# CILAB-MA/gpudrive_lab

Hardware: AMD Instinct MI355X
Metric: agent-steps/sec at 1024 worlds x 64 agents; achieved HBM GB/s on obs kernel (higher is better)
Workload: dtype f32

## Files before the change

### gpudrive_lab_amd/csrc/engine.cpp

```cpp
#include <hip/hip_runtime.h>

#include <algorithm>
#include <cmath>
#include <cstdlib>
#include <cstdio>
#include <cstring>
#include <map>
#include <memory>
#include <stdexcept>
#include <atomic>
#include <exception>
#include <string>
#include <thread>
#include <vector>

#include "engine.hpp"
#include "gd_math.hpp"
#include "scene.hpp"
#ifdef GD_CLOCKS
namespace gd { void set_clocks_read(unsigned long long *out); void step_clocks_read(unsigned long long *out); }
#endif
#ifndef GD_GRID_MIN_CELL
#define GD_GRID_MIN_CELL 16.f
#endif
// ... 100 lines not shown
    size_t lin_cap = 0;
    int32_t *d_row_of_slot = nullptr, *d_slot_of_row = nullptr, *d_row_count = nullptr;
    int32_t *d_lin_list = nullptr, *d_lin_list_dyn = nullptr;
    std::vector<std::vector<int32_t>> w_resp;
    bool full_pass_next = false;
    int64_t lin_static_agents = 0;
    int64_t host_skipped = 0;
    bool rk_possible = false;
    bool rk_alloc = false;

    bool ensure_rank_buffers() {
        if (rk_alloc) return true;
        const size_t WA = static_cast<size_t>(W) * A;
        const size_t first = internal.size();
        try {
            if (std::getenv("GPUDRIVE_RANK_ALLOC_FAIL") != nullptr) {
                d.rk_E = alloc_internal<uint16_t>(WA * GD_RANK_CAP + 64);
                d.rk_spc = alloc_internal<uint16_t>(WA * GD_RANK_SPL);
                throw HipError("GPUDRIVE_RANK_ALLOC_FAIL: simulated allocation failure of the rank replay's buffers");
            }
            d.rk_E = alloc_internal<uint16_t>(WA * GD_RANK_CAP + 64);
            d.rk_spc = alloc_internal<uint16_t>(WA * GD_RANK_SPL);
            d.rk_kt = alloc_internal<float>(WA * GD_RANK_KT);
            d.rk_heap = alloc_internal<uint32_t>(WA * GD_RANK_HEAP_DW);
            d.rk_cpe = alloc_internal<uint16_t>(WA * GD_RANK_NCP);
            d.rk_n = alloc_internal<int32_t>(WA);
            d.rk_fallback = alloc_internal<int32_t>(WA / 32);
            d.rk_streak = alloc_internal<int32_t>(WA / 32);
            d.cp_road = alloc_internal<uint16_t>(2 * WA * GD_RANK_NCP);
            d.cp_T = alloc_internal<float>(2 * WA * GD_RANK_NCP);
            d.cp_hdr = alloc_internal<float4>(2 * WA);
            d.rk_words = alloc_internal<uint32_t>(WA * GD_RANK_NCH);
            d.rk_tl = alloc_internal<float>(WA);
            d.rk_hist = alloc_internal<int32_t>(544);
            d.rk_ticket = alloc_internal<int32_t>(WA);
            d.rk_order = alloc_internal<int32_t>(WA);
            d.rk_list = alloc_internal<int32_t>(8 * WA);
            d.rk_nlong = static_cast<int>(std::max<size_t>(WA / 4, 64));
            d.rk_longlist = alloc_internal<int32_t>(d.rk_nlong);
            d.rk_longslot = alloc_internal<int32_t>(WA);
            d.rk_E_long = alloc_internal<uint16_t>(static_cast<size_t>(d.rk_nlong) * GD_RANK_CAP_LONG + 64);
            d.rk_kt_long = alloc_internal<float>(static_cast<size_t>(d.rk_nlong) * GD_RANK_KT_LONG);
        } catch (const HipError &) {
            (void)hipGetLastError();
            for (size_t k = first; k < internal.size(); k++) (void)hipFree(internal[k]);
            internal.resize(first);
            rk_possible = false;
            d.rk_on = 0;
            d.rk_nlong = 0;
            d.rk_E = nullptr; d.rk_spc = nullptr; d.rk_kt = nullptr; d.rk_heap = nullptr; d.rk_cpe = nullptr; d.rk_n = nullptr;
            d.rk_fallback = nullptr; d.rk_streak = nullptr; d.cp_road = nullptr; d.cp_T = nullptr; d.cp_hdr = nullptr;
            d.rk_words = nullptr; d.rk_tl = nullptr; d.rk_hist = nullptr; d.rk_ticket = nullptr; d.rk_order = nullptr;
            d.rk_list = nullptr; d.rk_longlist = nullptr; d.rk_longslot = nullptr; d.rk_E_long = nullptr; d.rk_kt_long = nullptr;
            return false;
        }
        rk_alloc = true;
        return true;
    }
    bool timing = false;
    std::vector<EventPair> ev_pool[gd::KERNEL_TIMED];
    size_t ev_head[gd::KERNEL_TIMED] = {};
    size_t ev_used[gd::KERNEL_TIMED] = {};
    double ev_ms[gd::KERNEL_TIMED] = {};
    int64_t ev_launches[gd::KERNEL_TIMED] = {};

    ~gd_sim() {
        (void)hipDeviceSynchronize();
// ... 49 lines not shown
    void launch(int which, bool move, hipStream_t stream_override = nullptr) {
        hipStream_t stream = stream_override ? stream_override : this->stream;
        const bool timed = timing && which < gd::KERNEL_TIMED && !d.gate_any;
        EventPair ep{};
        if (timed) {
            if (ev_used[which] == ev_pool[which].size()) collect_timing(which, ev_pool[which].size() / 2);
            ep = ev_pool[which][(ev_head[which] + ev_used[which]) % ev_pool[which].size()];
            ev_used[which]++;
            HIP_CHECK(hipEventRecord(ep.start, stream));
        }
        if (which == gd::KERNEL_BEV) gd::launch_bev(d, stream);
        else if (which == gd::KERNEL_LIDAR) gd::launch_lidar(d, stream);
        else gd::launch_kernel(d, stream, which, move);
        if (timed) HIP_CHECK(hipEventRecord(ep.stop, stream));
        HIP_CHECK(hipGetLastError());
    }

    hipGraphExec_t step_graph = nullptr;
    int64_t stat_graph_steps = 0, stat_plain_steps = 0, stat_captures = 0;
    bool graph_ok = std::getenv("GPUDRIVE_NO_GRAPH") == nullptr;

    void drop_graph() {
        if (step_graph) {
            (void)hipGraphExecDestroy(step_graph);
            step_graph = nullptr;
        }
    }

    void choose_set_schedule() {
        d.set_apw = 2;
        d.set_fused_rows = 1;
        if (const char *e = std::getenv("GPUDRIVE_SET_FUSED_ROWS")) d.set_fused_rows = std::atoi(e) != 0 ? 1 : 0;
        if (const char *e = std::getenv("GPUDRIVE_SET_AGENTS_PER_WAVE")) d.set_apw = std::min(32, std::max(1, std::atoi(e)));
    }

    void step() {
        if (full_pass_next) {
            full_pass_next = false;
            d.lin_dyn_off = 1;
            d.bev_all_dirty = 1;
            try {
                run_rest(true);
            } catch (...) {
                d.lin_dyn_off = 0;
                d.bev_all_dirty = 0;
                throw;
            }
            d.lin_dyn_off = 0;
            d.bev_all_dirty = 0;
            stat_plain_steps++;
            return;
        }
        if (params.roadObservationAlgorithm != GD_ROADS_K_NEAREST && d.lin_on && d.pose_skip && !params.disableClassicalObs)
            host_skipped += lin_static_agents;
        if (!graph_ok || timing || stream == nullptr) {
            run_rest(true);
            stat_plain_steps++;
            return;
        }
        if (!step_graph) {
            hipGraph_t g = nullptr;
            if (hipStreamBeginCapture(stream, hipStreamCaptureModeThreadLocal) != hipSuccess) {
                (void)hipGetLastError();
                graph_ok = false;
                run_rest(true);
                return;
// ... 509 lines not shown
        std::vector<int32_t> co(ncell);
        std::vector<uint16_t> ci(nitem);
        std::vector<float> cxy(nitem * 2);
        std::vector<uint16_t> cpos(nitem);
        for (int w = 0; w < W; w++) {
            std::copy(w_rcell_off[w].begin(), w_rcell_off[w].end(), co.begin() + w_rgrid[w].cell_base);
            std::copy(w_rcell_items[w].begin(), w_rcell_items[w].end(), ci.begin() + w_rgrid[w].item_base);
            for (size_t k = 0; k < w_rcell_items[w].size(); k++) {
                const size_t r = w_rcell_items[w][k], o = (static_cast<size_t>(w_rgrid[w].item_base) + k) * 2;
                cxy[o] = w_xy[w][2 * r];
                cxy[o + 1] = w_xy[w][2 * r + 1];
                cpos[static_cast<size_t>(w_rgrid[w].item_base) + r] = static_cast<uint16_t>(k);
            }
        }
        if (ncell) HIP_CHECK(hipMemcpy(d_rcell_off, co.data(), ncell * sizeof(int32_t), hipMemcpyHostToDevice));
        if (nitem) HIP_CHECK(hipMemcpy(d_rcell_items, ci.data(), nitem * sizeof(uint16_t), hipMemcpyHostToDevice));
        if (nitem) HIP_CHECK(hipMemcpy(d_rcell_xy, cxy.data(), nitem * 2 * sizeof(float), hipMemcpyHostToDevice));
        if (nitem) HIP_CHECK(hipMemcpy(d_rcell_pos, cpos.data(), nitem * sizeof(uint16_t), hipMemcpyHostToDevice));
        d.rcell_xy = static_cast<const float2 *>(d_rcell_xy);
        d.rcell_pos = static_cast<const uint16_t *>(d_rcell_pos);
        HIP_CHECK(hipMemcpy(const_cast<gd::GridHdr *>(d.rgrid), w_rgrid.data(), sizeof(gd::GridHdr) * W, hipMemcpyHostToDevice));
        d.rcell_off = static_cast<const int32_t *>(d_rcell_off);
        d.rcell_items = static_cast<const uint16_t *>(d_rcell_items);
        std::vector<float> prev(static_cast<size_t>(W) * A * 4, 0.f);
        for (size_t i = 0; i < static_cast<size_t>(W) * A; i++) prev[i * 4 + 2] = INFINITY;
        HIP_CHECK(hipMemcpy(d.knn_prev, prev.data(), prev.size() * sizeof(float), hipMemcpyHostToDevice));
    }

    void reset_rank_state() {
        HIP_CHECK(hipMemset(d.cp_hdr, 0, sizeof(float4) * 2 * static_cast<size_t>(W) * A));
        HIP_CHECK(hipMemset(d.rk_fallback, 0, sizeof(int32_t) * (static_cast<size_t>(W) * A / 32)));
        HIP_CHECK(hipMemset(d.rk_streak, 0, sizeof(int32_t) * (static_cast<size_t>(W) * A / 32)));
        HIP_CHECK(hipMemset(d.rk_hist, 0, sizeof(int32_t) * GD_RANK_AUDIT));
    }

    void do_reset(const std::vector<int32_t> &flags) {
        upload_flags(d.reset_flags, flags);
        reset_flagged(false);
    }

    void reset_flagged(bool gated) {
        d.gate_any = gated ? 1 : 0;
        if (!gated) full_pass_next = false;
        try {
            launch(gd::KERNEL_RESET, false);
            run_rest(false);
        } catch (...) {
            d.gate_any = 0;
            throw;
        }
        d.gate_any = 0;
    }
};

namespace {

template <typename F>
int guarded(F &&f) {
    try {
        f();
        return GD_OK;
    } catch (const HipError &e) {
        return fail(GD_ERR_DEVICE, e.what());
    } catch (const std::invalid_argument &e) {
        const std::string m = e.what();
        return fail(m.find("cannot open") != std::string::npos ? GD_ERR_IO : GD_ERR_INVALID, m);
// ... 62 lines not shown
        s->w_boxes.resize(W);
        s->w_grid.resize(W);
        s->w_cell_off.resize(W);
        s->w_cell_items.resize(W);
        s->w_rgrid.resize(W);
        s->w_rcell_off.resize(W);
        s->w_rcell_items.resize(W);
        for (int id = 0; id < GD_T_COUNT; id++) {
            if (id == GD_T_BEV && !cfg->alloc_bev && !cfg->external[id]) continue;
            const int64_t bytes = spec_bytes(tensor_spec(id, W, A));
            if (cfg->external[id]) {
                s->exported[id] = cfg->external[id];
            } else {
                HIP_CHECK(hipMalloc(&s->exported[id], bytes));
                s->owned[id] = true;
            }
            HIP_CHECK(hipMemset(s->exported[id], 0, bytes));
        }
        gd::DevSim &d = s->d;
        d.W = W;
        d.A = A;
        d.p = *params;
        d.knn_order = cfg->knn_order;
        d.split_partner = (s->stream != nullptr && std::getenv("GPUDRIVE_SPLIT_PARTNER") != nullptr) ? 1 : 0;
        HIP_CHECK(hipStreamCreateWithFlags(&s->side, hipStreamNonBlocking));
        HIP_CHECK(hipEventCreateWithFlags(&s->ev_fork, hipEventDisableTiming));
        HIP_CHECK(hipEventCreateWithFlags(&s->ev_join, hipEventDisableTiming));
        d.step_dbg = 0;
#ifdef GD_DIAG
        if (const char *e = std::getenv("GPUDRIVE_STEP_DBG")) d.step_dbg = std::atoi(e);
#endif
        {
            (void)hipDeviceGetAttribute(&s->cu_count, hipDeviceAttributeMultiprocessorCount, cfg->device_id);
            d.set_fused_rows = 0;
            d.set_apw = 16;
        }
        d.lidar_half_angle = cfg->lidar_half_angle;
        {
            const float r = params->observationRadius;
            float k = r * r;
            while (k > 0.f && sqrtf(k) > r) k = std::nextafterf(k, 0.f);
            while (sqrtf(std::nextafterf(k, INFINITY)) <= r) k = std::nextafterf(k, INFINITY);
            d.radius_key_max = r >= 0.f ? k : -1.f;
        }
        d.action = static_cast<float *>(s->exported[GD_T_ACTION]);
        d.reward = static_cast<float *>(s->exported[GD_T_REWARD]);
        d.done = static_cast<int32_t *>(s->exported[GD_T_DONE]);
        d.info = static_cast<int32_t *>(s->exported[GD_T_INFO]);
        d.self_obs = static_cast<float *>(s->exported[GD_T_SELF_OBS]);
        d.abs_obs = static_cast<float *>(s->exported[GD_T_ABS_OBS]);
        d.partner = static_cast<float *>(s->exported[GD_T_PARTNER_OBS]);
        d.agent_map = static_cast<float *>(s->exported[GD_T_AGENT_MAP_OBS]);
        d.map_obs = static_cast<float *>(s->exported[GD_T_MAP_OBS]);
        d.lidar = static_cast<float *>(s->exported[GD_T_LIDAR]);
        d.bev = static_cast<float *>(s->exported[GD_T_BEV]);
        d.steps = static_cast<uint32_t *>(s->exported[GD_T_STEPS_REMAINING]);
        d.shape = static_cast<int32_t *>(s->exported[GD_T_SHAPE]);
        d.controlled = static_cast<int32_t *>(s->exported[GD_T_CONTROLLED_STATE]);
        d.resp_export = static_cast<int32_t *>(s->exported[GD_T_RESPONSE_TYPE]);
        d.traj = static_cast<float *>(s->exported[GD_T_EXPERT_TRAJECTORY]);
        d.means = static_cast<float *>(s->exported[GD_T_WORLD_MEANS]);
        d.metadata = static_cast<int32_t *>(s->exported[GD_T_METADATA]);
        d.deleted = static_cast<int32_t *>(s->exported[GD_T_DELETED_AGENTS]);
        d.map_name = static_cast<int32_t *>(s->exported[GD_T_MAP_NAME]);
        d.scenario_id = static_cast<int32_t *>(s->exported[GD_T_SCENARIO_ID]);
        const size_t WA = static_cast<size_t>(W) * A;
// ... 419 lines not shown
    });
}

int gd_stat(gd_sim *s, int32_t which, int64_t *out) {
#ifdef GD_CLOCKS
    if (s && out && which >= 22 && which <= 29) {
        static unsigned long long clk[8];
        if (which == 22) gd::set_clocks_read(clk);
        *out = (int64_t)clk[which - 22];
        return GD_OK;
    }
#endif
#ifdef GD_CLOCKS
    if (s && out && which >= 32 && which <= 43) {
        static unsigned long long clk[12];
        if (which == 32) gd::step_clocks_read(clk);
        *out = (int64_t)clk[which - 32];
        return GD_OK;
    }
#endif
#ifdef GD_CLOCKS
    if (s && out && which >= 1000 && which < 1256) {
        *out = 0;
        if (s->rk_alloc) {
            int32_t v = 0;
            (void)hipStreamSynchronize(s->stream);
            if (hipMemcpy(&v, s->d.rk_hist + 256 + (which - 1000), sizeof(v), hipMemcpyDeviceToHost) != hipSuccess)
                return fail(GD_ERR_DEVICE, "gd_stat: reading the replay clocks failed");
            *out = v;
        }
        return GD_OK;
    }
#endif
#if defined(GD_DIAG) || defined(GD_CLOCKS)
    constexpr int32_t kLastStat = 20;
#else
    constexpr int32_t kLastStat = 7;
#endif
    if (s && out && which == 30) {
        std::vector<unsigned long long> v(GD_SKIP_SLOTS, 0);
        (void)hipStreamSynchronize(s->stream);
        if (hipMemcpy(v.data(), s->d.stat_skipped, sizeof(unsigned long long) * v.size(), hipMemcpyDeviceToHost) != hipSuccess ||
            hipMemset(s->d.stat_skipped, 0, sizeof(unsigned long long) * v.size()) != hipSuccess)
            return fail(GD_ERR_DEVICE, "gd_stat: reading the skip counters failed");
        unsigned long long sum = 0;
        for (unsigned long long x : v) sum += x;
        *out = static_cast<int64_t>(sum) + s->host_skipped;
        s->host_skipped = 0;
        return GD_OK;
    }
    if (s && out && which == 31) {
        int32_t c = 0;
        (void)hipStreamSynchronize(s->stream);
        if (hipMemcpy(&c, s->d.bev_count, sizeof(c), hipMemcpyDeviceToHost) != hipSuccess)
            return fail(GD_ERR_DEVICE, "gd_stat: reading the raster count failed");
        *out = c;
        return GD_OK;
    }
    if (s && out && which == 44) {
        std::vector<int32_t> f(static_cast<size_t>(s->W) * s->A), n(static_cast<size_t>(s->W) * 2);
        (void)hipStreamSynchronize(s->stream);
        if (hipMemcpy(f.data(), s->d.lidar_dirty, sizeof(int32_t) * f.size(), hipMemcpyDeviceToHost) != hipSuccess ||
            hipMemcpy(n.data(), s->d.shape, sizeof(int32_t) * n.size(), hipMemcpyDeviceToHost) != hipSuccess)
            return fail(GD_ERR_DEVICE, "gd_stat: reading the LiDAR flags failed");
        int64_t c = 0;
        for (int w = 0; w < s->W; w++)
            for (int a = 0; a < n[static_cast<size_t>(w) * 2] && a < s->A; a++) c += f[static_cast<size_t>(w) * s->A + a] != 0;
        *out = c;
        return GD_OK;
    }
    if (s && out && which == 45) {
        unsigned long long v = 0;
        (void)hipStreamSynchronize(s->stream);
        if (hipMemcpy(&v, s->d.bad_actions, sizeof(v), hipMemcpyDeviceToHost) != hipSuccess)
            return fail(GD_ERR_DEVICE, "gd_stat: reading the action counter failed");
        *out = static_cast<int64_t>(v);
        return GD_OK;
    }
    if (s && out && which == 46) {
        unsigned long long v = 0;
        (void)hipStreamSynchronize(s->stream);
        if (hipMemcpy(&v, s->d.warm_count, sizeof(v), hipMemcpyDeviceToHost) != hipSuccess)
            return fail(GD_ERR_DEVICE, "gd_stat: reading the warm-up counter failed");
        *out = static_cast<int64_t>(v);
        return GD_OK;
    }
    if (s && out && which == 21) {
        *out = 0;
        if (s->rk_alloc) {
            int32_t v = 0;
            (void)hipStreamSynchronize(s->stream);
            if (hipMemcpy(&v, s->d.rk_hist + GD_RANK_AUDIT, sizeof(v), hipMemcpyDeviceToHost) != hipSuccess)
                return fail(GD_ERR_DEVICE, "gd_stat: reading the audit counter failed");
            *out = v;
        }
        return GD_OK;
    }
    if (!s || !out || which < 0 || which > kLastStat) return fail(GD_ERR_INVALID, "gd_stat: bad argument");
#if defined(GD_DIAG) || defined(GD_CLOCKS)
    if (which >= 8) {
        *out = 0;
        if (s->rk_alloc) {
            int32_t v = 0;
            (void)hipStreamSynchronize(s->stream);
            (void)hipMemcpy(&v, s->d.rk_hist + 514 + (which - 8), sizeof(v), hipMemcpyDeviceToHost);
            (void)hipMemset(s->d.rk_hist + 514 + (which - 8), 0, sizeof(v));
            *out = v;
        }
        return GD_OK;
    }
#endif
    if (which == 7) {
        *out = s->d.rk_on;
        return GD_OK;
    }
    *out = which == 0 ? s->stat_graph_steps : which == 1 ? s->stat_plain_steps : which == 2 ? s->stat_captures
         : which == 3 ? s->d.set_fused_rows : which == 4 ? s->d.set_apw : which == 5 ? s->d.live_count : GD_MAP_OBS_AW;
// ... 152 lines not shown
```

### gpudrive_lab_amd/csrc/engine.hpp

```cpp
#pragma once
#include <hip/hip_runtime.h>

#include <cstdint>

#include "../../include/gpudrive_amd.h"

#ifndef GD_MAP_OBS_AW
#define GD_MAP_OBS_AW 32
#endif

#define GD_RANK_CAP 1280
#define GD_RANK_NCP 40
#define GD_RANK_HEAP_DW 104
#define GD_RANK_CAP_LONG 2560
#define GD_RANK_KT_LONG 164
#define GD_RH_LONG 537
#define GD_RANK_NCH 320
#define GD_RANK_SPL 256
#define GD_RANK_KT 84
#define GD_RANK_AUDIT 536
#define GD_LIN_BLK 16
#define GD_SKIP_SLOTS 4096

#ifdef GD_DIAG
#define GD_DIAG_IS(field, value) ((field) == (value))
#else
#define GD_DIAG_IS(field, value) false
#endif

namespace gd {

enum { KERNEL_STATE = 0, KERNEL_MAP_OBS = 1, KERNEL_LIDAR = 2, KERNEL_BEV = 3, KERNEL_PARTNER = 4, KERNEL_RESET = 5, KERNEL_PADDING = 6, KERNEL_TIMED = 5 };

struct GridHdr {
    float ox, oy, inv_cell;
    int nx, ny;
    int cell_base;
    int item_base;
    int pad;
};

struct DevSim {
    int W, A;
    int knn_order;
    int set_fused_rows;
    int32_t *live_list;
    int live_count;
    int32_t *set_groups;
    int set_group_count;
    int set_apw;
    float lidar_half_angle;
    float radius_key_max;
    gd_params p;
// ... 26 lines not shown
    const int32_t *rcell_off;
    const uint16_t *rcell_items;
    const float2 *rcell_xy;
    const uint16_t *rcell_pos;
    float4 *knn_prev;
    const int32_t *lin_list, *lin_list_dyn;
    int lin_blocks, lin_blocks_dyn;
    int lin_dyn_off;
    const float4 *road_blk;
    const int32_t *blk_off;
    int lin_apw;
    int lin_on;
    uint4 *pose_stamp;
    int pose_skip;
    int32_t *bev_dirty;
    int32_t *bev_list;
    int32_t *bev_count;
    int bev_all_dirty;
    int32_t *lidar_dirty;
    float *lidar_head;
    float *pack;
    int pack_only;
    const int32_t *row_of_slot, *slot_of_row;
    int n_rows;
    int pack_rows;
    unsigned long long *bad_actions;
    unsigned long long *stat_skipped;
    int split_partner;
    int step_dbg;
    int rk_on;
    int rk_max_roads;
    int rk_min_roads;
    int rk_dbg;
    uint16_t *rk_E;
    int rk_nlong;
    int32_t *rk_longlist;
    int32_t *rk_longslot;
    uint16_t *rk_E_long;
    float *rk_kt_long;
    uint16_t *rk_spc;
    float *rk_kt;
    uint32_t *rk_heap;
    uint16_t *rk_cpe;
    int32_t *rk_hist;
    int32_t *rk_ticket;
    int32_t *rk_order;
    int32_t *rk_list;
    uint32_t *rk_words;
    float *rk_tl;
    const float4 *road_bbox;
    const float *road_rbmax;
    int32_t *rk_n;
    int32_t *rk_fallback;
    int32_t *rk_streak;
    uint16_t *cp_road;
    float *cp_T;
    float4 *cp_hdr;
    int warm_k;
    int warm_all;
    int32_t *warm_flags;
    unsigned long long *warm_count;
    const float *pack_weights;
};

void launch_kernel(const DevSim &d, hipStream_t st, int which, bool move);
void launch_map_obs(const DevSim &d, hipStream_t st, bool move);
void launch_map_obs_rank(const DevSim &d, hipStream_t st);
void launch_map_obs_linear(const DevSim &d, hipStream_t st, bool move);
void launch_bev(const DevSim &d, hipStream_t st);
void launch_lidar(const DevSim &d, hipStream_t st);
void launch_pack_obs(const DevSim &d, hipStream_t st, float *out);
void launch_expert_actions(const DevSim &d, hipStream_t st, float *actions, float *pos, float *vel, float *yaw, int *valid);
void launch_set_log_actions(const DevSim &d, hipStream_t st, int t);
void launch_episode_step(const DevSim &d, hipStream_t st, const gd_episode_config &c, const gd_episode_buffers &b);
void launch_draw_weights(const DevSim &d, hipStream_t st, const gd_episode_config &c, const gd_episode_buffers &b,
                         const int32_t *worlds, int n);
void launch_pack_obs_rows(const DevSim &d, hipStream_t st, float *out,
                          const float *weights);
void launch_learner_rows(hipStream_t st, const uint8_t *mask, size_t slots, int32_t *row_of_slot, int32_t *slot_of_row,
                         int32_t *count);
void launch_discrete_actions(const DevSim &d, hipStream_t st, const int64_t *indices, const float *table, int n_actions);
void launch_pack_obs_conditioned(const DevSim &d, hipStream_t st, const float *weights, float *out);
void launch_record(const DevSim &d, hipStream_t st, const gd_record_buffers &b, int t, bool pre);

}
```

### gpudrive_lab_amd/csrc/map_obs_rank.hip

```cpp
#include <hip/hip_runtime.h>

#include <algorithm>
#include <type_traits>

#include "engine.hpp"
#include "gd_math.hpp"
#include "rank_heap.hpp"

namespace gd {

namespace {

constexpr int K = GD_MAP_OBS_K;
constexpr int CAP = GD_RANK_CAP;
constexpr int NCP = GD_RANK_NCP;
constexpr int SPL = GD_RANK_SPL;
constexpr int KT = GD_RANK_KT;
constexpr int TILE = 32;
constexpr int CAP_LONG = GD_RANK_CAP_LONG;
template <int CAP_T>
struct RankGeo {
    static constexpr bool LONG = CAP_T > CAP;
    static constexpr int NG = CAP_T / 64;
    static constexpr int NMAX = CAP_T - 8;
// ... 308 lines not shown
    }
    if (wave == 0 && ranked != 0ull) {
        list_base = __builtin_amdgcn_readfirstlane(list_base);
        if (ncp > 0)
            d.rk_list[(size_t)(blockIdx.x & 7) * WA + audited(d, list_base + __popcll(ranked & ((1ull << lane) - 1ull)), (int)WA)] = (int)i;
    }
}

template <int CAP_T>
struct RankLds {
    union {
        unsigned short cidx[CAP_T];
        struct {
            float skey[CAP_T];
            unsigned short spos[CAP_T];
        } s;
        unsigned short spc[CAP_T];
    };
    unsigned int cnt2[RankGeo<CAP_T>::NB / 2];
};
static_assert(sizeof(RankLds<CAP>) <= 10240 && sizeof(RankLds<CAP_LONG>) <= 20480, "sixteen / eight waves per CU");

constexpr int WPL = GD_RANK_NCH / 64;
struct RankIn {
    int i, state, r0, R, li;
    float ex, ey, iw, iz, t_last;
    unsigned int wd[WPL];
};
template <typename T>
__device__ __forceinline__ T uniform_load(const T *p) {
    return *reinterpret_cast<const __attribute__((address_space(4))) T *>(reinterpret_cast<uintptr_t>(p));
}
template <int A_T>
__device__ __forceinline__ RankIn rank_fetch(const DevSim &d, const int *list, int li, int count, int lane) {
    RankIn in;
    in.li = li;
    in.i = li < count ? uniform_load(list + li) : 0;
    in.state = li < count ? uniform_load(d.rk_n + in.i) : 0;
    const int w = in.i / A_T;
    in.r0 = uniform_load(d.road_off + w);
    in.R = uniform_load(d.road_off + w + 1) - in.r0;
    in.ex = uniform_load(d.px + in.i); in.ey = uniform_load(d.py + in.i);
    in.iw = uniform_load(d.qw + in.i); in.iz = -uniform_load(d.qz + in.i);
    in.t_last = uniform_load(d.rk_tl + in.i);
    const int nch = (in.R + 31) >> 5;
    const uint32_t *words = d.rk_words + (size_t)in.i * GD_RANK_NCH;
#pragma unroll
    for (int k = 0; k < WPL; k++) {
        const int c = k * 64 + lane;
        in.wd[k] = (in.state == 1 && c < nch) ? (GD_NT_WORDS_LOAD ? stream_load(words + c) : words[c]) : 0u;
    }
    return in;
}

#ifdef GD_CLOCKS
struct PhaseClock {
    unsigned int prev, sum[8];
    __device__ __forceinline__ void mark(int n) {
        const unsigned int t = (unsigned int)__builtin_amdgcn_s_memtime();
        sum[n] += t - prev;
        prev = t;
    }
};
#define GD_PHASE(n) clk.mark(n)
#else
struct PhaseClock {};
#define GD_PHASE(n)
#endif
template <int A_T, int CAP_T>
__device__ __forceinline__ void rank_agent(const DevSim &d, const RankIn &in, int lane, RankLds<CAP_T> &L, PhaseClock &clk, int next_entry,
                                           int count, const int *list, RankIn &nxt) {
    using G = RankGeo<CAP_T>;
    constexpr int NB = G::NB, NLIN = G::NLIN, NMAX = G::NMAX;
    constexpr unsigned int TM = (1u << G::RSH) - 1u;
    if (__builtin_amdgcn_readfirstlane(in.state) != 1) {
        nxt = rank_fetch<A_T>(d, list, next_entry, count, lane);
        return;
    }
    auto uni = [](int v) -> int { return __builtin_amdgcn_readfirstlane(v); };
    auto unif = [](float v) -> float { return __int_as_float(__builtin_amdgcn_readfirstlane(__float_as_int(v))); };
    const int i = uni(in.i), r0 = uni(in.r0), R = uni(in.R);
    const int group = i / 32;
    constexpr int NG = G::NG;

    const int nch = (R + 31) >> 5;
    {
        int mine = 0;
#pragma unroll
        for (int k = 0; k < WPL; k++) {
            const int c = k * 64 + lane;
            unsigned int wd = k * 64 < nch ? in.wd[k] : 0u;
            if (k == 0) wd = c < K / 32 ? 0u : (c == K / 32 ? wd & ~((1u << (K % 32)) - 1u) : wd);
            mine += __popc(wd);
        }
        const int total = K + wave_sum(mine);
        if (total > NMAX) {
            if (lane == 0) {
                bool passed_on = false;
                if (!G::LONG && total <= RankGeo<CAP_LONG>::NMAX) {
                    const int slot = atomicAdd(&d.rk_hist[GD_RH_LONG], 1);
                    if (slot < d.rk_nlong) {
                        d.rk_longlist[slot] = i;
                        passed_on = true;
                    }
                }
                if (!passed_on) {
                    d.rk_n[i] = 0;
                    d.rk_ticket[i] = -3;
                    d.rk_fallback[group] = 1;
                }
            }
            nxt = rank_fetch<A_T>(d, list, next_entry, count, lane);
            return;
        }
    }

    static_assert(K == 200 && CAP >= 256, "roads 0..K-1: four stores per lane");
#pragma unroll
    for (int q = 0; q < 4; q++)
        if (q * 64 + lane < K) L.cidx[q * 64 + lane] = (unsigned short)(q * 64 + lane);
    int nin = K;
#pragma unroll
    for (int k = 0; k < WPL; k++) {
        if (k * 64 >= nch) break;
        const int c = k * 64 + lane;
        unsigned int wd = in.wd[k];
        if (k == 0) wd = c < K / 32 ? 0u : (c == K / 32 ? wd & ~((1u << (K % 32)) - 1u) : wd);
        const int pc = __popc(wd);
#ifdef GD_CLOCKS
        clk.sum[7] += (unsigned int)wave_max(pc) << 8;
#endif
        const int incl = wave_incl_scan(pc);
        int pos = nin + incl - pc;
        nin += __builtin_amdgcn_readlane(incl, 63);
        while (wd) {
            L.cidx[pos++] = (unsigned short)((c << 5) + __ffs(wd) - 1);
            wd &= wd - 1u;
        }
    }
    wave_sync();
    const int bin = 255 - min(255, (nin - K) / 5);
    int ticket = 0;
    if (lane == 0) ticket = bin << 20 | atomicAdd(&d.rk_hist[bin], 1);
    GD_PHASE(1);
    if (GD_DIAG_IS(d.rk_dbg, 1)) {
        nxt = rank_fetch<A_T>(d, list, next_entry, count, lane);
        return;
    }
    if (lane <= (nin - K) >> G::TSH) {
        const int road = (int)L.cidx[K - 1 + (lane << G::TSH)];
        d.cp_road[(size_t)i * NCP + lane] = (unsigned short)(lane ? min(65535, (road + 1 + 31) & ~31) : (K / 32) * 32);
    }
    constexpr int GQ = 5;
    static_assert(NG % GQ == 0, "whole groups");
    int ci[NG];
#pragma unroll
    for (int g0 = 0; g0 < NG; g0 += GQ) {
#pragma unroll
        for (int u = 0; u < GQ; u++) ci[g0 + u] = 0;
        if (g0 * 64 < nin) {
            int v[GQ];
#pragma unroll
            for (int u = 0; u < GQ; u++) v[u] = (int)L.cidx[(g0 + u) * 64 + lane];
#pragma unroll
            for (int u = 0; u < GQ; u++) ci[g0 + u] = (g0 + u) * 64 + lane < nin ? v[u] : 0;
        }
    }
    wave_sync();
    const float ex = unif(in.ex), ey = unif(in.ey), iw = unif(in.iw), iz = unif(in.iz);
    const float kmax = d.radius_key_max;
    const float2 *rxy = d.road_xy + r0;
    float key[NG];
    const float t_last = unif(in.t_last);
    float split = (t_last > 0.f && t_last < 1e30f) ? t_last * 1.5f : 1.f;
    int nle = 0, nlow = 0;
    float kmax_seen = 0.f, kmin_seen = __builtin_inff();
#pragma unroll
    for (int g0 = 0; g0 < NG; g0 += GQ) {
#pragma unroll
        for (int u = 0; u < GQ; u++) key[g0 + u] = 0.f;
        if (g0 * 64 < nin) {
            float2 xy[GQ];
#pragma unroll
            for (int u = 0; u < GQ; u++) xy[u] = rxy[(unsigned int)ci[g0 + u]];
            static_assert(GQ == 5, "operand list");
            asm volatile("" : "+v"(xy[0].x), "+v"(xy[0].y), "+v"(xy[1].x), "+v"(xy[1].y), "+v"(xy[2].x), "+v"(xy[2].y),
                              "+v"(xy[3].x), "+v"(xy[3].y), "+v"(xy[4].x), "+v"(xy[4].y));
#pragma unroll
            for (int u = 0; u < GQ; u++) {
                const int g = g0 + u;
                key[g] = ego_dist2(ex, ey, iw, iz, xy[u].x, xy[u].y);
                const bool on = g * 64 + lane < nin;
                nle += ((on & (key[g] <= kmax)) ? 1 : 0) + ((on & (key[g] < split)) ? 1 << 16 : 0);
                kmax_seen = fmaxf(kmax_seen, on ? key[g] : 0.f);
                kmin_seen = fminf(kmin_seen, on ? key[g] : __builtin_inff());
            }
        }
    }
    nxt = rank_fetch<A_T>(d, list, next_entry, count, lane);
    nle = wave_sum(nle);
    kmax_seen = wave_max_nonneg(kmax_seen);
    kmin_seen = wave_min_nonneg(kmin_seen);
    nlow = nle >> 16;
    nle &= 0xffff;
    GD_PHASE(2);
    if (GD_DIAG_IS(d.rk_dbg, 2)) return;

    for (int b = lane; b < NB / 2; b += 64) L.cnt2[b] = 0u;
    wave_sync();
    const bool jumped = nlow * 4 < nin || nlow == nin;
    const float lin_lo = jumped ? kmin_seen : 0.f;
    const int nlin = jumped ? NB : NLIN;
    const float lin_scale = jumped ? (float)NB / fmaxf(kmax_seen - kmin_seen, 1e-30f) : (float)NLIN / split;
    if (jumped) split = __builtin_inff();
    const unsigned int split_bits = __float_as_uint(split);
    const float log_scale = (float)(NB - NLIN) / (float)(max(__float_as_uint(kmax_seen), split_bits + 1u) - split_bits + 1u);
    auto bucket_of = [&](float k) -> int {
        if (k < split) return min(nlin - 1, max(0, (int)((k - lin_lo) * lin_scale)));
        return NLIN + min(NB - NLIN - 1, (int)((float)(__float_as_uint(k) - split_bits) * log_scale));
    };
#pragma unroll
    for (int g = 0; g < NG; g++) {
        if (g * 64 < nin) {
            const int b = bucket_of(key[g]);
            ci[g] |= b << 16;
            if (g * 64 + lane < nin) atomicAdd(&L.cnt2[b >> 1], 1u << ((b & 1) * 16));
        }
    }
    wave_sync();
    {
        constexpr int WPB = NB / 64 / 2;
        static_assert(WPB * 128 == NB, "whole counter words per lane");
// ... 137 lines not shown
    }
    unsigned short *const E_row = G::LONG ? d.rk_E_long + (size_t)uni(in.li) * CAP_LONG : d.rk_E + (size_t)i * CAP;
    const unsigned int ulane = (unsigned int)lane;
#pragma unroll
    for (int g = 0; g < NG; g++) {
        if (g * 64 < nin) {
            if (g * 64 + lane < nin) {
                const unsigned int e = (unsigned int)ci[g] >> 16;
                stream_store((unsigned short)e, E_row + (g * 64u + ulane));
                const int slot = (int)(e >> G::RSH) - 1 + (int)(e & TM);
                if (slot < SPL) L.spc[slot] = (unsigned short)(ci[g] & 0xffff);
            }
        }
    }
    wave_sync();
    {
        static_assert(SPL == 256, "four slots per lane");
        const uint2 v = reinterpret_cast<const uint2 *>(L.spc)[lane];
        stream_store(v, reinterpret_cast<uint2 *>(d.rk_spc + (size_t)i * SPL) + ulane);
    }
    if (lane == 0) {
        d.rk_n[i] = nin | (nle << 16) | (has_tie ? 1 << 28 : 0) | (G::LONG ? 1 << 29 : 0);
        if (G::LONG) d.rk_longslot[i] = uni(in.li);
        d.rk_ticket[i] = ticket;
    }
    GD_PHASE(6);
}

template <int A_T, int CAP_T>
__global__ __launch_bounds__(64, CAP_T > CAP ? 2 : 4) void k_knn_rank(DevSim d) {
    if (d.gate_any && *d.any_reset == 0) return;
    __shared__ RankLds<CAP_T> L;
    constexpr bool LONG = RankGeo<CAP_T>::LONG;
    const int stride = LONG ? (int)gridDim.x : (int)(gridDim.x >> 3);
    const int xcd = blockIdx.x & 7;
    const int count = LONG ? min(uniform_load(d.rk_hist + GD_RH_LONG), d.rk_nlong) : uniform_load(d.rk_hist + 528 + xcd);
    const int *list = LONG ? d.rk_longlist : d.rk_list + (size_t)xcd * d.W * A_T;
    int t = LONG ? (int)blockIdx.x : (int)(blockIdx.x >> 3);
    RankIn cur = rank_fetch<A_T>(d, list, t, count, threadIdx.x);
    PhaseClock clk;
#ifdef GD_CLOCKS
    for (int k = 0; k < 8; k++) clk.sum[k] = 0u;
    clk.prev = (unsigned int)__builtin_amdgcn_s_memtime();
#endif
    for (; t < count; t += stride) {
        RankIn nxt;
        GD_PHASE(0);
        rank_agent<A_T, CAP_T>(d, cur, threadIdx.x, L, clk, t + stride, count, list, nxt);
        wave_sync();
        cur = nxt;
    }
#ifdef GD_CLOCKS
    if (threadIdx.x == 0)
        for (int k = 0; k < 8; k++) atomicAdd(reinterpret_cast<unsigned int *>(&d.rk_hist[516 + k]), clk.sum[k] >> 8);
#endif
}

#ifndef GD_RANK_AWR
#define GD_RANK_AWR 64
#endif
constexpr int AWR = GD_RANK_AWR;
typedef unsigned int __attribute__((may_alias)) heap_u32;
typedef unsigned short __attribute__((may_alias)) heap_u16;
struct RankHeap {
    heap_u32 *pr;
    __device__ __forceinline__ unsigned int pair(int j) const { return pr[j * AWR]; }
    __device__ __forceinline__ unsigned int get(int g) const {
        return reinterpret_cast<const heap_u16 *>(pr + (g >> 1) * AWR)[g & 1];
    }
    __device__ __forceinline__ void set(int g, unsigned int v) const {
        reinterpret_cast<heap_u16 *>(pr + (g >> 1) * AWR)[g & 1] = (unsigned short)v;
    }
    __device__ __forceinline__ void set_pair(int j, unsigned int v) const { pr[j * AWR] = v; }
};
static_assert(rank_heap::NPAIR == 128, "s_pair of k_knn_replay");

__global__ __launch_bounds__(256) void k_knn_order(DevSim d) {
    if (d.gate_any && *d.any_reset == 0) return;
    __shared__ int s_part[4];
    __shared__ int s_start[256];
    const int tl = threadIdx.x;
    const int c = d.rk_hist[tl];
    const int incl = wave_incl_scan(c);
    if ((tl & 63) == 63) s_part[tl >> 6] = incl;
    __syncthreads();
    int before = 0;
    for (int k = 0; k < (tl >> 6); k++) before += s_part[k];
    s_start[tl] = before + incl - c;
    if (blockIdx.x == 0 && tl == 255) {
        d.rk_hist[512] = before + incl;
        d.rk_hist[513]++;
        for (int x = 0; x < 8; x++) d.rk_hist[528 + x] = 0;
        d.rk_hist[GD_RH_LONG] = 0;
    }
#ifdef GD_CLOCKS
    if (blockIdx.x == 0) d.rk_hist[256 + tl] = 0;
#endif
    __syncthreads();
    const int t = blockIdx.x * 256 + tl;
    if (t >= d.live_count) return;
    const int i = d.live_list[t];
    const int ticket = d.rk_ticket[i];
    if (ticket < 0) return;
    d.rk_order[audited(d, s_start[(ticket >> 20) & 255] + (ticket & 0xfffff), d.W * d.A)] = i;
}

#ifdef GD_CLOCKS
struct ReplayClock {
    unsigned int prev, first, ph[5];
    __device__ __forceinline__ void start() { first = prev = (unsigned int)__builtin_amdgcn_s_memrealtime(); }
    __device__ __forceinline__ void mark(int n) {
        const unsigned int t = (unsigned int)__builtin_amdgcn_s_memrealtime();
        ph[n] = t - prev;
        prev = t;
    }
};
#define GD_RPHASE(n) rclk.mark(n)
#else
#define GD_RPHASE(n)
#endif
__global__ __launch_bounds__(64) void k_knn_replay(DevSim d) {
    if (d.gate_any && *d.any_reset == 0) return;
    const int lane = threadIdx.x;
#ifdef GD_CLOCKS
    ReplayClock rclk;
    rclk.start();
#endif
    if (blockIdx.x == 0)
        for (int k = 0; k < 4; k++) d.rk_hist[k * 64 + lane] = 0;
// ... 283 lines not shown
        }
    }
    wave_sync();
#pragma unroll
    for (int ps = 0; ps < NP; ps++) {
        const int q = ps * 64 + lane;
        if (q < K) {
            const unsigned int v = q < m ? s_sorted[wave][q] : (unsigned int)q << 16;
            d.sel_idx[(size_t)i * K + q] = (unsigned short)(v & 0xffffu);
            d.sel_slot[(size_t)i * K + q] = (unsigned char)(v >> 16);
        }
    }
    const bool at_start = steps_left == (uint32_t)GD_EPISODE_LEN;
    const size_t WA = (size_t)d.W * A_T;
    if (lane < ncp) {
        (void)audited(d, cp_slot, n);
        d.cp_T[(size_t)i * NCP + lane] = cp_t;
        if (at_start) {
            d.cp_T[(WA + i) * NCP + lane] = cp_t;
            d.cp_road[(WA + i) * NCP + lane] = cp_r;
        }
    }
    if (lane == 0) {
        d.rk_streak[i / 32] = 0;
        d.cp_hdr[i] = make_float4(ex, ey, __int_as_float(ncp), 0.f);
        if (at_start) d.cp_hdr[WA + i] = make_float4(ex, ey, __int_as_float(ncp), 0.f);
        d.sel_hdr[(size_t)i * 2] = make_float4(ex, ey, qw, qz);
        d.sel_hdr[(size_t)i * 2 + 1] = make_float4(__int_as_float(m), __int_as_float(r0), __int_as_float(1), 0.f);
    }
}

}

#ifndef GD_RANK_LONG_GRID
#define GD_RANK_LONG_GRID 2048
#endif
void launch_map_obs_rank(const DevSim &d, hipStream_t st) {
    if (d.live_count == 0) return;
    const dim3 glong(std::min(std::max(d.rk_nlong, 1), GD_RANK_LONG_GRID));
    const dim3 gr(std::min((d.live_count + 7) / 8 * 8, 256 * 8 * 4)), g4((d.live_count + 3) / 4), gw(d.W * (d.A / 64));
    if (d.A == 64) {
        hipLaunchKernelGGL((k_knn_scan<64>), gw, dim3(256), 0, st, d);
        hipLaunchKernelGGL((k_knn_rank<64, CAP>), gr, dim3(64), 0, st, d);
        if (d.rk_nlong > 0) hipLaunchKernelGGL((k_knn_rank<64, CAP_LONG>), glong, dim3(64), 0, st, d);
    } else {
        hipLaunchKernelGGL((k_knn_scan<128>), gw, dim3(256), 0, st, d);
        hipLaunchKernelGGL((k_knn_rank<128, CAP>), gr, dim3(64), 0, st, d);
        if (d.rk_nlong > 0) hipLaunchKernelGGL((k_knn_rank<128, CAP_LONG>), glong, dim3(64), 0, st, d);
    }
    hipLaunchKernelGGL(k_knn_order, dim3((d.live_count + 255) / 256), dim3(256), 0, st, d);
    hipLaunchKernelGGL(k_knn_replay, dim3((d.live_count + AWR - 1) / AWR), dim3(64), 0, st, d);
    if (d.A == 64) hipLaunchKernelGGL((k_knn_finish<64>), g4, dim3(256), 0, st, d);
    else hipLaunchKernelGGL((k_knn_finish<128>), g4, dim3(256), 0, st, d);
}

}
```

Before: 63.60 million.

## Use atomic work queues with cross-XCD stealing and occupancy-sized grids in rank kernel

The rank kernel's static grid-stride split over the per-XCD agent lists is replaced by a dynamic queue. Each wave draws its next entry with an atomic counter, and once its home list is drained it steals from the other XCDs' lists. The grid size now comes from occupancy queries times CU count instead of fixed constants. The aim is to remove load imbalance and tail latency between XCD lists, at the cost of an atomic per agent, extra counter bookkeeping in rk_hist, and new diagnostic stats.

```diff
diff --git a/gpudrive_lab_amd/csrc/engine.cpp b/gpudrive_lab_amd/csrc/engine.cpp
--- a/gpudrive_lab_amd/csrc/engine.cpp
+++ b/gpudrive_lab_amd/csrc/engine.cpp
@@ -156,7 +156,7 @@
             d.cp_hdr = alloc_internal<float4>(2 * WA);
             d.rk_words = alloc_internal<uint32_t>(WA * GD_RANK_NCH);
             d.rk_tl = alloc_internal<float>(WA);
-            d.rk_hist = alloc_internal<int32_t>(544);
+            d.rk_hist = alloc_internal<int32_t>(GD_RH_SIZE);
             d.rk_ticket = alloc_internal<int32_t>(WA);
             d.rk_order = alloc_internal<int32_t>(WA);
             d.rk_list = alloc_internal<int32_t>(8 * WA);
@@ -272,6 +272,18 @@
         d.set_fused_rows = 1;
         if (const char *e = std::getenv("GPUDRIVE_SET_FUSED_ROWS")) d.set_fused_rows = std::atoi(e) != 0 ? 1 : 0;
         if (const char *e = std::getenv("GPUDRIVE_SET_AGENTS_PER_WAVE")) d.set_apw = std::min(32, std::max(1, std::atoi(e)));
+    }
+
+    void choose_rank_grid() {
+        auto waves = [&](bool long_list, int fallback_per_cu, const char *pin_name) {
+            int per_cu = gd::rank_waves_per_cu(A, long_list);
+            if (per_cu <= 0) per_cu = fallback_per_cu;
+            int n = per_cu * cu_count * (long_list ? 1 : GD_RANK_GRID_X);
+            if (const char *pin = std::getenv(pin_name)) n = std::max(1, std::atoi(pin));
+            return n;
+        };
+        d.rk_grid = (waves(false, 16, "GPUDRIVE_RANK_WAVES") + 7) / 8 * 8;
+        d.rk_grid_long = waves(true, 8, "GPUDRIVE_RANK_LONG_WAVES");
     }
 
     void step() {
@@ -847,6 +859,7 @@
         HIP_CHECK(hipMemset(d.rk_fallback, 0, sizeof(int32_t) * (static_cast<size_t>(W) * A / 32)));
         HIP_CHECK(hipMemset(d.rk_streak, 0, sizeof(int32_t) * (static_cast<size_t>(W) * A / 32)));
         HIP_CHECK(hipMemset(d.rk_hist, 0, sizeof(int32_t) * GD_RANK_AUDIT));
+        HIP_CHECK(hipMemset(d.rk_hist + GD_RH_LONG, 0, sizeof(int32_t) * (GD_RH_SIZE - GD_RH_LONG)));
     }
 
     void do_reset(const std::vector<int32_t> &flags) {
@@ -975,6 +988,7 @@
 #endif
         {
             (void)hipDeviceGetAttribute(&s->cu_count, hipDeviceAttributeMultiprocessorCount, cfg->device_id);
+            s->choose_rank_grid();
             d.set_fused_rows = 0;
             d.set_apw = 16;
         }
@@ -1460,6 +1474,19 @@
         return GD_OK;
     }
 #endif
+#ifdef GD_CLOCKS
+    if (s && out && which >= 1300 && which < 1364) {
+        *out = 0;
+        if (s->rk_alloc) {
+            uint32_t v = 0;
+            (void)hipStreamSynchronize(s->stream);
+            if (hipMemcpy(&v, s->d.rk_hist + GD_RH_TAIL_LAST + (which - 1300), sizeof(v), hipMemcpyDeviceToHost) != hipSuccess)
+                return fail(GD_ERR_DEVICE, "gd_stat: reading the ranking's tail failed");
+            *out = v;
+        }
+        return GD_OK;
+    }
+#endif
 #if defined(GD_DIAG) || defined(GD_CLOCKS)
     constexpr int32_t kLastStat = 20;
 #else
@@ -1511,6 +1538,21 @@
         if (hipMemcpy(&v, s->d.warm_count, sizeof(v), hipMemcpyDeviceToHost) != hipSuccess)
             return fail(GD_ERR_DEVICE, "gd_stat: reading the warm-up counter failed");
         *out = static_cast<int64_t>(v);
+        return GD_OK;
+    }
+    if (s && out && which >= 47 && which <= 49) {
+        *out = 0;
+        if (s->rk_alloc) {
+            int32_t v = 0;
+            (void)hipStreamSynchronize(s->stream);
+            if (hipMemcpy(&v, s->d.rk_hist + GD_RH_DONE_LAST + (which - 47), sizeof(v), hipMemcpyDeviceToHost) != hipSuccess)
+                return fail(GD_ERR_DEVICE, "gd_stat: reading the ranking's entry counts failed");
+            *out = v;
+        }
+        return GD_OK;
+    }
+    if (s && out && (which == 50 || which == 51)) {
+        *out = which == 50 ? s->d.rk_grid : s->d.rk_grid_long;
         return GD_OK;
     }
     if (s && out && which == 21) {
diff --git a/gpudrive_lab_amd/csrc/engine.hpp b/gpudrive_lab_amd/csrc/engine.hpp
--- a/gpudrive_lab_amd/csrc/engine.hpp
+++ b/gpudrive_lab_amd/csrc/engine.hpp
@@ -19,6 +19,19 @@
 #define GD_RANK_SPL 256
 #define GD_RANK_KT 84
 #define GD_RANK_AUDIT 536
+#define GD_RH_DRAW 576
+#define GD_RH_DRAW_LONG 832
+#define GD_RH_DONE 538
+#define GD_RH_DONE_LONG 539
+#define GD_RH_DONE_LAST 540
+#define GD_RH_LISTED_LAST 541
+#define GD_RH_DONE_LONG_LAST 542
+#define GD_RH_TAIL 896
+#define GD_RH_TAIL_LAST 960
+#define GD_RH_SIZE 1024
+#ifndef GD_RANK_GRID_X
+#define GD_RANK_GRID_X 1
+#endif
 #define GD_LIN_BLK 16
 #define GD_SKIP_SLOTS 4096
 
@@ -111,6 +124,7 @@
     int rk_max_roads;
     int rk_min_roads;
     int rk_dbg;
+    int rk_grid, rk_grid_long;
     uint16_t *rk_E;
     int rk_nlong;
     int32_t *rk_longlist;
@@ -145,6 +159,7 @@
 void launch_kernel(const DevSim &d, hipStream_t st, int which, bool move);
 void launch_map_obs(const DevSim &d, hipStream_t st, bool move);
 void launch_map_obs_rank(const DevSim &d, hipStream_t st);
+int rank_waves_per_cu(int agent_slots, bool long_list);
 void launch_map_obs_linear(const DevSim &d, hipStream_t st, bool move);
 void launch_bev(const DevSim &d, hipStream_t st);
 void launch_lidar(const DevSim &d, hipStream_t st);
diff --git a/gpudrive_lab_amd/csrc/map_obs_rank.hip b/gpudrive_lab_amd/csrc/map_obs_rank.hip
--- a/gpudrive_lab_amd/csrc/map_obs_rank.hip
+++ b/gpudrive_lab_amd/csrc/map_obs_rank.hip
@@ -364,11 +364,11 @@
     return *reinterpret_cast<const __attribute__((address_space(4))) T *>(reinterpret_cast<uintptr_t>(p));
 }
 template <int A_T>
-__device__ __forceinline__ RankIn rank_fetch(const DevSim &d, const int *list, int li, int count, int lane) {
+__device__ __forceinline__ RankIn rank_fetch(const DevSim &d, const int *list, int li, bool valid, int lane) {
     RankIn in;
     in.li = li;
-    in.i = li < count ? uniform_load(list + li) : 0;
-    in.state = li < count ? uniform_load(d.rk_n + in.i) : 0;
+    in.i = valid ? uniform_load(list + li) : 0;
+    in.state = valid ? uniform_load(d.rk_n + in.i) : 0;
     const int w = in.i / A_T;
     in.r0 = uniform_load(d.road_off + w);
     in.R = uniform_load(d.road_off + w + 1) - in.r0;
@@ -385,6 +385,46 @@
     return in;
 }
 
+template <int A_T, bool LONG>
+struct RankQueue {
+    static constexpr int NL = LONG ? 1 : 8;
+    int home, s;
+    int count;
+    const int *list;
+    int *ctr;
+    int done, stolen;
+    __device__ __forceinline__ void open(const DevSim &d, int x) {
+        count = LONG ? min(uniform_load(d.rk_hist + GD_RH_LONG), d.rk_nlong) : uniform_load(d.rk_hist + 528 + x);
+        list = LONG ? d.rk_longlist : d.rk_list + (size_t)x * d.W * A_T;
+        ctr = d.rk_hist + (LONG ? GD_RH_DRAW_LONG : GD_RH_DRAW + 32 * x);
+    }
+    __device__ __forceinline__ void init(const DevSim &d, int xcd) {
+        home = xcd; s = 0; done = 0; stolen = 0;
+        open(d, xcd);
+    }
+    __device__ __forceinline__ bool live() const { return s < NL; }
+    __device__ __forceinline__ int reserve(int lane) const {
+        int t = 0;
+        if (live() && lane == 0) t = atomicAdd(ctr, 1);
+        return t;
+    }
+    __device__ __forceinline__ int take(const DevSim &d, int reserved, int lane) {
+        int t = __builtin_amdgcn_readfirstlane(reserved);
+        while (live() && t >= count) {
+            s++;
+            if (live()) {
+                open(d, (home + s) & 7);
+                t = __builtin_amdgcn_readfirstlane(reserve(lane));
+            }
+        }
+        return t;
+    }
+    __device__ __forceinline__ RankIn fetch(const DevSim &d, int reserved, int lane) {
+        const int t = take(d, reserved, lane);
+        return rank_fetch<A_T>(d, list, t, live(), lane);
+    }
+};
+
 #ifdef GD_CLOCKS
 struct PhaseClock {
     unsigned int prev, sum[8];
@@ -400,13 +440,13 @@
 #define GD_PHASE(n)
 #endif
 template <int A_T, int CAP_T>
-__device__ __forceinline__ void rank_agent(const DevSim &d, const RankIn &in, int lane, RankLds<CAP_T> &L, PhaseClock &clk, int next_entry,
-                                           int count, const int *list, RankIn &nxt) {
+__device__ __forceinline__ void rank_agent(const DevSim &d, const RankIn &in, int lane, RankLds<CAP_T> &L, PhaseClock &clk,
+                                           RankQueue<A_T, RankGeo<CAP_T>::LONG> &q, RankIn &nxt) {
     using G = RankGeo<CAP_T>;
     constexpr int NB = G::NB, NLIN = G::NLIN, NMAX = G::NMAX;
     constexpr unsigned int TM = (1u << G::RSH) - 1u;
     if (__builtin_amdgcn_readfirstlane(in.state) != 1) {
-        nxt = rank_fetch<A_T>(d, list, next_entry, count, lane);
+        nxt = q.fetch(d, q.reserve(lane), lane);
         return;
     }
     auto uni = [](int v) -> int { return __builtin_amdgcn_readfirstlane(v); };
@@ -442,7 +482,7 @@
                     d.rk_fallback[group] = 1;
                 }
             }
-            nxt = rank_fetch<A_T>(d, list, next_entry, count, lane);
+            nxt = q.fetch(d, q.reserve(lane), lane);
             return;
         }
     }
@@ -474,9 +514,10 @@
     const int bin = 255 - min(255, (nin - K) / 5);
     int ticket = 0;
     if (lane == 0) ticket = bin << 20 | atomicAdd(&d.rk_hist[bin], 1);
+    const int drawn = q.reserve(lane);
     GD_PHASE(1);
     if (GD_DIAG_IS(d.rk_dbg, 1)) {
-        nxt = rank_fetch<A_T>(d, list, next_entry, count, lane);
+        nxt = q.fetch(d, drawn, lane);
         return;
     }
     if (lane <= (nin - K) >> G::TSH) {
@@ -529,7 +570,7 @@
             }
         }
     }
-    nxt = rank_fetch<A_T>(d, list, next_entry, count, lane);
+    nxt = q.fetch(d, drawn, lane);
     nle = wave_sum(nle);
     kmax_seen = wave_max_nonneg(kmax_seen);
     kmin_seen = wave_min_nonneg(kmin_seen);
@@ -733,27 +774,45 @@
     if (d.gate_any && *d.any_reset == 0) return;
     __shared__ RankLds<CAP_T> L;
     constexpr bool LONG = RankGeo<CAP_T>::LONG;
-    const int stride = LONG ? (int)gridDim.x : (int)(gridDim.x >> 3);
-    const int xcd = blockIdx.x & 7;
-    const int count = LONG ? min(uniform_load(d.rk_hist + GD_RH_LONG), d.rk_nlong) : uniform_load(d.rk_hist + 528 + xcd);
-    const int *list = LONG ? d.rk_longlist : d.rk_list + (size_t)xcd * d.W * A_T;
-    int t = LONG ? (int)blockIdx.x : (int)(blockIdx.x >> 3);
-    RankIn cur = rank_fetch<A_T>(d, list, t, count, threadIdx.x);
+    const int lane = threadIdx.x;
+#ifdef GD_CLOCKS
+    const unsigned int t_start = (unsigned int)__builtin_amdgcn_s_memrealtime();
+#endif
+    RankQueue<A_T, LONG> q;
+    q.init(d, LONG ? 0 : (int)(blockIdx.x & 7));
+    RankIn cur = q.fetch(d, q.reserve(lane), lane);
     PhaseClock clk;
 #ifdef GD_CLOCKS
     for (int k = 0; k < 8; k++) clk.sum[k] = 0u;
     clk.prev = (unsigned int)__builtin_amdgcn_s_memtime();
 #endif
-    for (; t < count; t += stride) {
+    while (q.live()) {
         RankIn nxt;
         GD_PHASE(0);
-        rank_agent<A_T, CAP_T>(d, cur, threadIdx.x, L, clk, t + stride, count, list, nxt);
+        q.done++;
+        q.stolen += q.s != 0 ? 1 : 0;
+        rank_agent<A_T, CAP_T>(d, cur, lane, L, clk, q, nxt);
         wave_sync();
         cur = nxt;
     }
-#ifdef GD_CLOCKS
-    if (threadIdx.x == 0)
+    if (lane == 0 && q.done > 0) atomicAdd(&d.rk_hist[LONG ? GD_RH_DONE_LONG : GD_RH_DONE], q.done);
+#ifdef GD_CLOCKS
+    if (lane == 0) {
         for (int k = 0; k < 8; k++) atomicAdd(reinterpret_cast<unsigned int *>(&d.rk_hist[516 + k]), clk.sum[k] >> 8);
+        if (!LONG) {
+            const unsigned int t_exit = (unsigned int)__builtin_amdgcn_s_memrealtime();
+            unsigned int *tail = reinterpret_cast<unsigned int *>(d.rk_hist + GD_RH_TAIL + 8 * q.home);
+            atomicMax(tail + 0, ~t_start);
+            if (q.done > 0) {
+                atomicMax(tail + 1, t_exit);
+                atomicAdd(tail + 2, 1u);
+                atomicAdd(tail + 3, (unsigned int)q.done);
+                atomicAdd(tail + 4, (unsigned int)q.stolen);
+                atomicAdd(tail + 5, t_exit - t_start);
+                atomicAdd(reinterpret_cast<unsigned long long *>(tail + 6), (unsigned long long)t_exit);
+            }
+        }
+    }
 #endif
 }
 
@@ -791,11 +850,26 @@
     if (blockIdx.x == 0 && tl == 255) {
         d.rk_hist[512] = before + incl;
         d.rk_hist[513]++;
-        for (int x = 0; x < 8; x++) d.rk_hist[528 + x] = 0;
+        int listed = 0;
+        for (int x = 0; x < 8; x++) {
+            listed += d.rk_hist[528 + x];
+            d.rk_hist[528 + x] = 0;
+            d.rk_hist[GD_RH_DRAW + 32 * x] = 0;
+        }
         d.rk_hist[GD_RH_LONG] = 0;
+        d.rk_hist[GD_RH_DRAW_LONG] = 0;
+        d.rk_hist[GD_RH_LISTED_LAST] = listed;
+        d.rk_hist[GD_RH_DONE_LAST] = d.rk_hist[GD_RH_DONE];
+        d.rk_hist[GD_RH_DONE_LONG_LAST] = d.rk_hist[GD_RH_DONE_LONG];
+        d.rk_hist[GD_RH_DONE] = 0;
+        d.rk_hist[GD_RH_DONE_LONG] = 0;
     }
 #ifdef GD_CLOCKS
     if (blockIdx.x == 0) d.rk_hist[256 + tl] = 0;
+    if (blockIdx.x == 0 && tl < 64) {
+        d.rk_hist[GD_RH_TAIL_LAST + tl] = d.rk_hist[GD_RH_TAIL + tl];
+        d.rk_hist[GD_RH_TAIL + tl] = 0;
+    }
 #endif
     __syncthreads();
     const int t = blockIdx.x * 256 + tl;
@@ -1145,13 +1219,24 @@
 
 }
 
-#ifndef GD_RANK_LONG_GRID
-#define GD_RANK_LONG_GRID 2048
-#endif
+int rank_waves_per_cu(int agent_slots, bool long_list) {
+    int n = 0;
+    const hipError_t e =
+        agent_slots == 64 ? (long_list ? hipOccupancyMaxActiveBlocksPerMultiprocessor(&n, k_knn_rank<64, CAP_LONG>, 64, 0)
+                                       : hipOccupancyMaxActiveBlocksPerMultiprocessor(&n, k_knn_rank<64, CAP>, 64, 0))
+                          : (long_list ? hipOccupancyMaxActiveBlocksPerMultiprocessor(&n, k_knn_rank<128, CAP_LONG>, 64, 0)
+                                       : hipOccupancyMaxActiveBlocksPerMultiprocessor(&n, k_knn_rank<128, CAP>, 64, 0));
+    if (e != hipSuccess) {
+        (void)hipGetLastError();
+        return 0;
+    }
+    return n;
+}
+
 void launch_map_obs_rank(const DevSim &d, hipStream_t st) {
     if (d.live_count == 0) return;
-    const dim3 glong(std::min(std::max(d.rk_nlong, 1), GD_RANK_LONG_GRID));
-    const dim3 gr(std::min((d.live_count + 7) / 8 * 8, 256 * 8 * 4)), g4((d.live_count + 3) / 4), gw(d.W * (d.A / 64));
+    const dim3 glong(std::min(std::max(d.rk_nlong, 1), d.rk_grid_long));
+    const dim3 gr(std::min((d.live_count + 7) / 8 * 8, d.rk_grid)), g4((d.live_count + 3) / 4), gw(d.W * (d.A / 64));
     if (d.A == 64) {
         hipLaunchKernelGGL((k_knn_scan<64>), gw, dim3(256), 0, st, d);
         hipLaunchKernelGGL((k_knn_rank<64, CAP>), gr, dim3(64), 0, st, d);
```

After: 62.88 million. 1.1% lower.
